# AlexandreGac/alphazero-chess

Measured on NVIDIA B200. Metric: mcts_simulations_per_sec, higher is better.
Workload: dtype bf16

## Files before the change

### alphazero-chess_b200/csrc/mcts.cu

```cuda
#include "mcts.h"
#include "nn.h"
#include "det_math.cuh"
#include <cstdio>
#include <cstring>
#include <algorithm>
#include <cmath>

namespace azb {

constexpr int WARPS = 4;

struct WarpShared {
    double gam[AZ_MAX_MOVES];
    float fval[AZ_MAX_MOVES];
    uint16_t moves[AZ_MAX_MOVES];
    uint16_t sidx[AZ_MAX_MOVES];
    DPos child;
    DPos key;
    int n_moves;
    int term;
    int has_ep;
    int pad;
};

__device__ __forceinline__ u64 rng_u64(u64 seed, u64 game, u64 ply, u64 stream, u64 counter) {
// ... 544 lines not shown
    move_step(x);
    return ColdOut{x.c, x.st_pos, x.st_games, x.st_sdepth};
}
__device__ __noinline__ ColdOut finish_game_cold(const SearchParams* prm, const SearchPtrs* ptr, WarpShared* sh, int g, GameCtl c) {
    Ctx x = cold_ctx(prm, ptr, sh, g, c);
    finish_game(x, __uint_as_float(c.park_scale));
    return ColdOut{x.c, x.st_pos, x.st_games, x.st_sdepth};
}
__device__ __noinline__ void root_noise_cold(const SearchParams* prm, const SearchPtrs* ptr, WarpShared* sh, int g, GameCtl c) {
    Ctx x = cold_ctx(prm, ptr, sh, g, c);
    apply_noise(x, 0, c.game_id, c.noise_ply);
}

#ifdef AZ_ADV_TIMING
#define ADV_T0() long long t_prev = clock64(), t_start = t_prev; unsigned long long t_acc[8] = {0, 0, 0, 0, 0, 0, 0, 0}
#define ADV_T(k) do { const long long t_now = clock64(); t_acc[k] += (unsigned long long)(t_now - t_prev); t_prev = t_now; } while (0)
#else
#define ADV_T0() do { } while (0)
#define ADV_T(k) do { } while (0)
#endif
template <int MINB>
__global__ void __launch_bounds__(WARPS * 32, MINB * 4 / WARPS) k_advance(const __grid_constant__ SearchParams prm, const __grid_constant__ SearchPtrs ptr) {
    __shared__ WarpShared shared[WARPS];
    const int g = (blockIdx.x * blockDim.x + threadIdx.x) >> 5;
    if (g >= prm.n_games) return;
    const uint2 path_spec = ptr.path[(size_t)g * prm.node_cap + min((int)(threadIdx.x & 31), prm.node_cap - 1)];
    Ctx x{prm, ptr, &shared[threadIdx.x >> 5], g, (int)(threadIdx.x & 31), (size_t)g * prm.node_cap, (size_t)g * prm.edge_cap,
          ptr.ctl[g], 0, 0, 0, 0, 0, 0, 0, 0, 0, 0, 0};
    if (g == 0 && x.lane == 0 && ptr.batch_zero) *ptr.batch_zero = 0;
    if (x.c.status != 0 && x.c.status != 4) return;
    if (!prm.consume && x.c.pending_node >= 0) return;

    ADV_T0();
    if (x.c.status == 4) {
        const ColdOut o = finish_game_cold(&prm, &ptr, x.sh, g, x.c);
        x.c = o.c; x.st_pos += o.st_pos; x.st_games += o.st_games; x.st_sdepth += o.st_sdepth;
    }
    const bool runnable = x.c.status == 0;
    if (runnable && x.c.pending_node >= 0) {
        const int node = x.c.pending_node, slot = x.c.pending_slot;
        const size_t off = x.ebase + ptr.node_edge_off[x.nbase + node];
        const int L = ptr.node_nedges[x.nbase + node];
        if (!prm.priors_scattered) {
            const float* pol = ptr.res_policy + (size_t)slot * AZ_ACTION_SPACE;
            for (int e = x.lane; e < L; e += 32) ptr.edge_P[off + e] = pol[ptr.edge_mv[off + e] >> 16];
        }
// ... 512 lines not shown
}

static void prof_mark_search(az_engine* e) {
    if (e->prof_every > 0 && e->stub_kind == 0 && e->cfg.precision != 1 && (e->prof_counter % (uint64_t)e->prof_every) == 0 &&
        !e->prof_adv_event) {
        cudaEventCreate(&e->prof_adv_event);
        cudaEventRecord(e->prof_adv_event, e->stream);
    }
}

static int run_wave(az_engine* e, SearchState* st) {
    const int blocks = (st->prm.n_games + WARPS - 1) / WARPS;
    st->prm.priors_scattered = (e->stub_kind == 0 && e->cfg.precision != 1) ? 1 : 0;
    if (st->prm.mode == 1) st->prm.cache_epoch = (uint32_t)((st->wave_counter++ / (unsigned long long)std::max(st->prm.S, 1)) & 63);
    st->batch_parity ^= 1;
    st->ptr.batch_count = st->batch_base + st->batch_parity;
    st->ptr.batch_zero = st->batch_base + (st->batch_parity ^ 1);
    prof_mark_search(e);
    const int passes = st->prm.mode == 1 && st->prm.cache_mask ? st->adv_passes : 1;
    for (int pass = 0; pass < passes; pass++) {
    st->prm.consume = pass == 0 ? 1 : 0;
    e->n_launches++;
    const int minb = e->knobs.adv_minb;
    switch (minb) {
        case 4: k_advance<4><<<blocks, WARPS * 32, 0, e->stream>>>(st->prm, st->ptr); break;
        case 5: k_advance<5><<<blocks, WARPS * 32, 0, e->stream>>>(st->prm, st->ptr); break;
        case 6: k_advance<6><<<blocks, WARPS * 32, 0, e->stream>>>(st->prm, st->ptr); break;
        case 7: k_advance<7><<<blocks, WARPS * 32, 0, e->stream>>>(st->prm, st->ptr); break;
        default: k_advance<3><<<blocks, WARPS * 32, 0, e->stream>>>(st->prm, st->ptr); break;
    }
    }
    st->prm.consume = 1;
    AZ_CUDA(e, cudaGetLastError());
    return evaluate_batch(e, st);
}

static int search_begin(az_engine* e, int n, const az_position* roots, const az_position* history, const uint32_t* hist_offsets,
                        int num_simulations, const uint64_t* noise_game_ids, const uint32_t* noise_plies, const float* visits_out,
                        SearchState& run) {
    SearchState* st = e->search;
    if (n < 0 || n > st->G) return set_err(e, AZ_ERR_CAPACITY, "more roots than az_config.max_games");
    if (n == 0) return 1;
    if (!roots || !visits_out) return set_err(e, AZ_ERR_INVALID_ARGUMENT, "null buffer");
    if (num_simulations <= 0 || num_simulations + 2 > st->prm.node_cap)
        return set_err(e, AZ_ERR_CAPACITY, "num_simulations exceeds az_config.num_simulations (pool size)");
    if (e->stub_kind == 0 && !e->net->loaded) return set_err(e, AZ_ERR_NO_WEIGHTS, "az_load_weights has not been called");
    cudaSetDevice(e->cfg.device);
    st->selfplay_active = false;
    SearchParams prm = st->prm;
    prm.n_games = n; prm.S = num_simulations; prm.mode = 0;
    run = *st;
    run.prm = prm;
    AZ_CUDA(e, cudaMemcpyAsync(e->d_wire, roots, (size_t)n * sizeof(az_position), cudaMemcpyHostToDevice, e->stream));
// ... 339 lines not shown
```

### alphazero-chess_b200/csrc/nn_heads_tc.cu

```cuda
#include "nn.h"
#include "tc_conv.cuh"
#include "device_once.h"
#include <algorithm>

namespace azb {
namespace htc {
constexpr int kStages = 3;
constexpr int kStageBytes = 32768;
constexpr int kOffA = 0;
constexpr int kW40Block = 48 * 128;
constexpr int kOffW40 = kOffA + kStages * kStageBytes;
constexpr int kOffW2 = kOffW40 + 2 * kW40Block;
constexpr int kOffP1 = kOffW2 + 64 * 64;
constexpr int kOffExp = kOffP1 + 2 * 8192;
constexpr int kV1Pitch = 520;
constexpr int kOffV1 = kOffExp + 4 * 16384;
constexpr int kOffMisc = kOffV1 + 32 * kV1Pitch * 2;
constexpr int kTotal = kOffMisc + 1024 + 1024;
constexpr int kGroupTiles = 16;
constexpr int kEpiThreads = 512;
constexpr int kThreads = 64 + kEpiThreads;
constexpr int kTmemCols = 512;
static_assert(kOffW40 % 1024 == 0 && kOffW2 % 1024 == 0 && kOffP1 % 1024 == 0 && kOffExp % 1024 == 0, "operand tiles must be 1024-byte aligned");
static_assert(kTotal <= 232448, "shared memory of one CTA");
// ... 83 lines not shown
    uint32_t* tmem_ptr_s = reinterpret_cast<uint32_t*>(wl1_full + 1);
    float* s_b40 = reinterpret_cast<float*>(misc + 160);
    float* s_b2 = reinterpret_cast<float*>(misc + 320);
    float* s_red = reinterpret_cast<float*>(misc + 576);
    float* s_vsum = reinterpret_cast<float*>(misc + 704);
    __nv_bfloat16* s_v1 = reinterpret_cast<__nv_bfloat16*>(smem + kOffV1);
    float* s_hid = reinterpret_cast<float*>(smem + kOffExp);

#ifdef AZ_HTC_TIMING
    long long tacc[20] = {}, tlast = clock64();
    const long long tbegin = tlast;
#endif
    const int t = threadIdx.x, warp = t >> 5, lane = t & 31;
    uint4 wreg[2] = {make_uint4(0, 0, 0, 0), make_uint4(0, 0, 0, 0)}, w2reg = make_uint4(0, 0, 0, 0);
#pragma unroll
    for (int u = 0; u < 2; u++) {
        const int i = t + u * kThreads;
        if (i < 40 * 16) wreg[u] = __ldg(reinterpret_cast<const uint4*>(w40) + i);
    }
    if (t < 64 * 4) w2reg = __ldg(reinterpret_cast<const uint4*>(wp2) + t);
    float breg = 0.0f;
    if (t < 40) breg = b40[t];
    else if (t >= 64 && t < 128) breg = bp2[t - 64];
    const int n = n_dev ? *n_dev : n_static;
    const int n_tiles = (n + 1) >> 1;
    const int my_tiles = (int)blockIdx.x < n_tiles ? (n_tiles - (int)blockIdx.x + (int)gridDim.x - 1) / (int)gridDim.x : 0;

    const int et = t - 64;
    const int ew = warp - 2;
    const int w = ew >> 3;
    const int q = warp & 3;
    const int cg = (ew & 7) >> 2;
    const int row = q * 32 + lane;
    const int bi = q >> 1, sq = row & 63;
    const int ti = (q & 1) + 2 * cg;
    const int tid128 = sq + 64 * cg;
    const int nw = (my_tiles - w + 1) >> 1;
    unsigned long long eo_cur = 0, eo_nxt = 0, eo_n2 = 0;
    int L_cur = 0, L_nxt = 0, L_n2 = 0;
    uint32_t mv_cur = 0, mv_nxt = 0;
    auto meta = [&](int j, unsigned long long& eo, int& L) {
        eo = 0; L = 0;
        if (sc.edge_P && j < nw) {
            const int b = ((int)blockIdx.x + (2 * j + w) * (int)gridDim.x) * 2 + bi;
            if (b < n) { eo = sc.edge_off[b]; L = sc.n_edges[b]; }
        }
    };
    if (warp >= 2) { meta(0, eo_cur, L_cur); meta(1, eo_nxt, L_nxt); }

    if (t == 0) {
        tma_prefetch_desc(&act_map);
        for (int i = 0; i < kStages; i++) { mbar_init(&a_full[i], 1); mbar_init(&a_empty[i], 1); }
        for (int i = 0; i < 2; i++) { mbar_init(&d1_full[i], 1); mbar_init(&p1_ready[i], 8); }
        for (int i = 0; i < 4; i++) { mbar_init(&d2_full[i], 1); mbar_init(&d2_free[i], 8); }
        mbar_init(wl1_full, 1);
        fence_barrier_init();
        for (int k = 0; k < kStages && k < my_tiles; k++) {
            const int tile = (int)blockIdx.x + k * (int)gridDim.x;
            mbar_arrive_expect_tx(&a_full[k], kStageBytes);
            tma1_load_2d(smem + kOffA + k * kStageBytes, &act_map, &a_full[k], 0, tile * 128);
            tma1_load_2d(smem + kOffA + k * kStageBytes + 16384, &act_map, &a_full[k], 64, tile * 128);
        }
    }
#pragma unroll
    for (int u = 0; u < 2; u++) {
        const int i = t + u * kThreads;
        if (i < 48 * 16) {
            const int r = i >> 4, ch = i & 15;
            *reinterpret_cast<uint4*>(smem + kOffW40 + (ch >> 3) * kW40Block + (r >> 3) * 1024 + (r & 7) * 128 + (((ch & 7) ^ (r & 7)) << 4)) = wreg[u];
        }
    }
    if (t < 64 * 4) {
        const int r = t >> 2, c = t & 3;
        *reinterpret_cast<uint4*>(smem + kOffW2 + (r >> 3) * 512 + (r & 7) * 64 + ((c ^ ((r >> 1) & 3)) << 4)) = w2reg;
    }
    if (t < 40) s_b40[t] = breg;
    if (t >= 64 && t < 128) s_b2[t - 64] = breg;
    fence_proxy_async_smem();
    if (warp == 1) tmem1_alloc(tmem_ptr_s, kTmemCols);
    tc_fence_before();
    __syncthreads();
    tc_fence_after();
    const uint32_t tmem_base = *tmem_ptr_s;
    HTC_T(0);

    if (warp == 0) {
        int stage = 0; uint32_t phase = 1;
        for (int k = kStages; k < my_tiles; k++) {
            const int tile = (int)blockIdx.x + k * (int)gridDim.x;
            mbar_wait(&a_empty[stage], phase ^ 1, 21);
            HTC_T(1);
            if (elect_one()) {
                mbar_arrive_expect_tx(&a_full[stage], kStageBytes);
                tma1_load_2d(smem + kOffA + stage * kStageBytes, &act_map, &a_full[stage], 0, tile * 128);
                tma1_load_2d(smem + kOffA + stage * kStageBytes + 16384, &act_map, &a_full[stage], 64, tile * 128);
            }
            __syncwarp();
            if (++stage == kStages) { stage = 0; phase ^= 1; }
        }
        if (my_tiles > 0 && my_tiles <= kGroupTiles) {
            for (int i = 0; i < kStages && i < my_tiles; i++) {
                mbar_wait(&a_empty[stage], phase ^ 1, 28);
                if (++stage == kStages) { stage = 0; phase ^= 1; }
            }
            if (elect_one()) {
                mbar_arrive_expect_tx(wl1_full, 64 * 1024);
// ... 220 lines not shown
    }
#ifdef AZ_HTC_TIMING
    if (blockIdx.x == 0 && lane == 0 && (warp <= 2 || warp == 10)) {
        const long long tot = clock64() - tbegin;
        printf("htc warp %d total %lld | setup %lld | p1 %lld p2 %lld p3 %lld p4 %lld p5 %lld p6 %lld p7 %lld p8 %lld p9 %lld p10 %lld p11 %lld p12 %lld p13 %lld p14 %lld p15 %lld | exp %lld shfl %lld\n", warp, tot,
               tacc[0], tacc[1], tacc[2], tacc[3], tacc[4], tacc[5], tacc[6], tacc[7], tacc[8], tacc[9], tacc[10], tacc[11], tacc[12], tacc[13], tacc[14], tacc[15], tacc[16], tacc[17]);
    }
#endif
    tc_fence_before();
    __syncthreads();
    if (warp == 1) { tc_fence_after(); tmem1_dealloc(tmem_base, kTmemCols); }
}

int launch_heads_tc(az_engine* e, const CUtensorMap* act_map, const int* n_dev, int n_static, float* policy_out, float* value_out,
                    const HeadScatter* scatter) {
    NetWeights* w = e->net;
    const int n_max = n_dev ? w->max_boards : n_static;
    if (n_max <= 0) return 0;
    const int grid = std::min((n_max + 1) / 2, e->sm_count);
    static PerDeviceOnce once;
    if (once.first()) cudaFuncSetAttribute(k_heads_tc, cudaFuncAttributeMaxDynamicSharedMemorySize, htc::kTotal);
    HeadScatter sc{nullptr, nullptr, nullptr, nullptr};
    if (scatter) sc = *scatter;
    k_heads_tc<<<grid, htc::kThreads, htc::kTotal, e->stream>>>(*act_map, w->h_w40, w->f_b40, w->h_wp2, w->f_bp2, w->h_wl1t, w->f_bl1, w->f_wl2,
                                                               w->f_bl2, policy_out, value_out, n_dev, n_static, sc);
    return check_cuda(e, cudaGetLastError(), "k_heads_tc");
}

}
```

### alphazero-chess_b200/csrc/nn_tc.cu

```cuda
#include "tc_conv.cuh"
#include "nn_tc.h"
#include "device_once.h"
#include <cuda_bf16.h>
#include <cstdio>
#include <cstdlib>

namespace azb {

constexpr int kWTileBytes = 64 * 128;

template <int HALVES, int KROW = 128, int WIDE = 0>
struct ConvSmem {
    static constexpr int kPitch = WIDE == 1 ? 16 : WIDE == 2 ? 10 : 8;
    static constexpr int kStages = HALVES == 1 ? 6 : WIDE == 1 ? 2 : WIDE == 2 ? 3 : 4;
    static constexpr int kWTiles = HALVES * 9;
    static constexpr int kStageB = 20 * kPitch * KROW;
    static constexpr int kWTileB = 64 * KROW;
    static constexpr int kWBytes = kWTiles * kWTileB;
    static constexpr int kABytes = kStages * kStageB;
    static constexpr int kMisc = 2048;
    static constexpr int kTotal = kWBytes + kABytes + kMisc + 1024;
};

constexpr int kTmemCols2 = 256;
// ... 11 lines not shown
__global__ void __cluster_dims__(2, 1, 1) __launch_bounds__(64 + GROUPS * kEpiThreads, 1)
conv3x3_tc2_kernel(const __grid_constant__ CUtensorMap in_map, const __grid_constant__ CUtensorMap w_map,
                   const float* __restrict__ bias, const __nv_bfloat16* __restrict__ residual,
                   __nv_bfloat16* __restrict__ out, const int* __restrict__ n_boards_ptr, int n_boards_static, int relu, int dbg) {
    using S = ConvSmem<HALVES, KROW, WIDE>;
    constexpr int kStageBytes = S::kStageB, kWTileBytes = S::kWTileB;
    constexpr int KSTEPS = KROW / 32;
    constexpr int NS = S::kStages;
    extern __shared__ uint8_t smem_raw[];
    uint8_t* smem = reinterpret_cast<uint8_t*>((reinterpret_cast<uintptr_t>(smem_raw) + 1023) & ~uintptr_t(1023));
    uint8_t* w_sm = smem;
    uint8_t* a_sm = smem + S::kWBytes;
    uint8_t* misc = a_sm + S::kABytes;
    float* bias_s = reinterpret_cast<float*>(misc);
    uint64_t* full_bar = reinterpret_cast<uint64_t*>(misc + 512);
    uint64_t* empty_bar = full_bar + NS;
    uint64_t* wfull_bar = empty_bar + NS;
    uint64_t* tfull_bar = wfull_bar + S::kWTiles;
    uint64_t* tempty_bar = tfull_bar + 2;
    uint32_t* tmem_ptr_s = reinterpret_cast<uint32_t*>(tempty_bar + 2);

    const int warp = threadIdx.x >> 5, lane = threadIdx.x & 31;
    const uint32_t rank = cluster_ctarank();
    const int n_boards = n_boards_ptr ? *n_boards_ptr : n_boards_static;
    const int n_tiles = (n_boards + 3) >> 2;
    const int first_tile = blockIdx.x >> 1, tile_step = gridDim.x >> 1;

    if (threadIdx.x == 0) {
        tma_prefetch_desc(&in_map);
        tma_prefetch_desc(&w_map);
        for (int i = 0; i < NS; i++) { mbar_init(&full_bar[i], 1); mbar_init(&empty_bar[i], 1); }
        for (int i = 0; i < S::kWTiles; i++) mbar_init(&wfull_bar[i], 1);
        for (int i = 0; i < 2; i++) { mbar_init(&tfull_bar[i], 1); mbar_init(&tempty_bar[i], 2 * kEpiWarps); }
        fence_barrier_init();
    }
    if (threadIdx.x >= 64 && threadIdx.x < 192) bias_s[threadIdx.x - 64] = bias[threadIdx.x - 64];
    if (warp == 1) tmem2_alloc(tmem_ptr_s, kTmemCols2);
    tc_fence_before();
    __syncthreads();
    cluster_sync_all();
    tc_fence_after();
    const uint32_t tmem_base = *tmem_ptr_s;

    if (warp == 0) {
        int stage = 0; uint32_t phase = 0; bool first = true;
        for (int t = first_tile; t < n_tiles; t += tile_step) {
            if constexpr (WIDE) {
                for (int half = 0; half < HALVES; half++) {
                    if (first && elect_one()) {
                        for (int dxi = 0; dxi < 3; dxi++)
                            for (int dyi = 0; dyi < 3; dyi++) {
                                const int wt = (half * 3 + dxi) * 3 + dyi, tap = dyi * 3 + dxi;
                                if (rank == 0) mbar_arrive_expect_tx(&wfull_bar[wt], 2 * kWTileBytes);
                                tma2_load_2d(w_sm + wt * kWTileBytes, &w_map, &wfull_bar[wt], half * 64, tap * 128 + (int)rank * 64);
                            }
                    }
                    mbar_wait(&empty_bar[stage], phase ^ 1, 11);
                    if (elect_one()) {
                        if (rank == 0) mbar_arrive_expect_tx(&full_bar[stage], 2 * kStageBytes);
                        tma2_load_4d(a_sm + stage * kStageBytes, &in_map, &full_bar[stage], half * 64, -1, t * 4 + (int)rank * 2, -1);
                    }
                    __syncwarp();
                    if (++stage == NS) { stage = 0; phase ^= 1; }
                }
                first = false;
            } else {
            for (int half = 0; half < HALVES; half++)
                for (int dxi = 0; dxi < 3; dxi++) {
                    if (first && elect_one()) {
                        for (int dyi = 0; dyi < 3; dyi++) {
                            const int wt = (half * 3 + dxi) * 3 + dyi, tap = dyi * 3 + dxi;
                            if (rank == 0) mbar_arrive_expect_tx(&wfull_bar[wt], 2 * kWTileBytes);
                            tma2_load_2d(w_sm + wt * kWTileBytes, &w_map, &wfull_bar[wt], half * 64, tap * 128 + (int)rank * 64);
                        }
                    }
                    mbar_wait(&empty_bar[stage], phase ^ 1, 11);
                    if (elect_one()) {
                        if (dbg & 1) { if (rank == 0) mbar_arrive(&full_bar[stage]); }
                        else {
                            if (rank == 0) mbar_arrive_expect_tx(&full_bar[stage], 2 * kStageBytes);
                            tma2_load_4d(a_sm + stage * kStageBytes, &in_map, &full_bar[stage], half * 64, dxi - 1, t * 4 + (int)rank * 2, -1);
                        }
                    }
                    __syncwarp();
                    if (++stage == NS) { stage = 0; phase ^= 1; }
                }
            first = false;
            }
        }
    } else if (warp == 1) {
        if (rank == 0) {
            constexpr uint32_t idesc = umma_idesc_bf16(256, 128);
            const uint64_t dbase = KROW == 128 ? umma_desc_base_sw128() : umma_desc_base_sw64();
            const uint32_t w_lo = (smem_u32(w_sm) & 0x3FFFF) >> 4;
            int stage = 0; uint32_t phase = 0; int lt = 0;
            for (int t = first_tile; t < n_tiles; t += tile_step, lt++) {
                const int acc = lt & 1; const uint32_t accphase = (lt >> 1) & 1;
                mbar_wait(&tempty_bar[acc], accphase ^ 1, 12);
                tc_fence_after();
                const uint32_t d_tmem = tmem_base + acc * 128;
                if constexpr (WIDE) {
                    for (int half = 0; half < HALVES; half++) {
                        mbar_wait(&full_bar[stage], phase, 13);
                        if (lt == 0)
                            for (int wt = 0; wt < 9; wt++) mbar_wait(&wfull_bar[half * 9 + wt], 0, 14);
                        tc_fence_after();
                        if (elect_one()) {
                            const uint32_t a_lo = (smem_u32(a_sm + stage * kStageBytes) & 0x3FFFF) >> 4;
                            const uint64_t abase = ((uint64_t)1 << 16) | ((uint64_t)((S::kPitch * KROW) >> 4) << 32) | ((uint64_t)1 << 46) | ((uint64_t)(KROW == 128 ? 2 : 4) << 61);
#pragma unroll
                            for (int dxi = 0; dxi < 3; dxi++) {
                                const uint32_t b_lo = w_lo + (uint32_t)((half * 3 + dxi) * 3) * (kWTileBytes >> 4);
// ... 132 lines not shown
template <int WIDE>
__global__ void __cluster_dims__(2, 1, 1) __launch_bounds__(kThreads2, 1)
conv_tower_kernel(const TowerParams prm) {
    using S = ConvSmem<2, 128, WIDE>;
    constexpr int kStageBytes = S::kStageB;
    constexpr int NS = S::kStages;
    constexpr int kGroupBytes = 3 * kWTileBytes;
    extern __shared__ uint8_t smem_raw[];
    uint8_t* smem = reinterpret_cast<uint8_t*>((reinterpret_cast<uintptr_t>(smem_raw) + 1023) & ~uintptr_t(1023));
    uint8_t* w_sm = smem;
    uint8_t* a_sm = smem + S::kWBytes;
    uint8_t* misc = a_sm + S::kABytes;
    uint64_t* full_bar = reinterpret_cast<uint64_t*>(misc);
    uint64_t* empty_bar = full_bar + NS;
    uint64_t* wfull_bar = empty_bar + NS;
    uint64_t* wempty_bar = wfull_bar + 6;
    uint64_t* tfull_bar = wempty_bar + 6;
    uint64_t* tempty_bar = tfull_bar + 2;
    uint32_t* tmem_ptr_s = reinterpret_cast<uint32_t*>(tempty_bar + 2);
    volatile uint32_t* epi_done = reinterpret_cast<volatile uint32_t*>(tmem_ptr_s + 4);

    const int warp = threadIdx.x >> 5, lane = threadIdx.x & 31;
    const uint32_t rank = cluster_ctarank();
    const int n_boards = prm.n_boards_ptr ? *prm.n_boards_ptr : prm.n_boards_static;
    const int n_tiles = min((n_boards + 3) >> 2, prm.tile_hi);
    const int tile_step = gridDim.x >> 1;
    const int n_ranges = n_tiles > prm.tile_lo ? (n_tiles - prm.tile_lo + prm.range_tiles - 1) / prm.range_tiles : 0;
#define TOWER_RANGE_BEGIN()                                                                                      \
    const int range_lo = prm.tile_lo + rg * prm.range_tiles;                                                      \
    const int range_hi = min(n_tiles, range_lo + prm.range_tiles);                                               \
    const int first_tile = range_lo + (blockIdx.x >> 1);                                                         \
    const int T = first_tile < range_hi ? (range_hi - first_tile + tile_step - 1) / tile_step : 0;               \
    if (T == 0) continue;
    const int stem = prm.stem;
    const int NL = prm.n_layers + stem;

    if (threadIdx.x == 0) {
        for (int i = 0; i < NS; i++) { mbar_init(&full_bar[i], 1); mbar_init(&empty_bar[i], 1); }
        for (int i = 0; i < 6; i++) { mbar_init(&wfull_bar[i], 1); mbar_init(&wempty_bar[i], 1); }
        for (int i = 0; i < 2; i++) { mbar_init(&tfull_bar[i], 1); mbar_init(&tempty_bar[i], 2 * kEpiWarps); }
        fence_barrier_init();
    }
    if (threadIdx.x < kEpiWarps) epi_done[threadIdx.x] = 0;
    float* bias_s = reinterpret_cast<float*>(misc + 512);
    if (warp == 1) tmem2_alloc(tmem_ptr_s, kTmemCols2);
    tc_fence_before();
    __syncthreads();
    cluster_sync_all();
    tc_fence_after();
    const uint32_t tmem_base = *tmem_ptr_s;

    if (warp == 0) {
        int stage = 0; uint32_t phase = 0;
        int u0 = 0, u1 = 0;
        uint32_t cum = 0;
        for (int rg = 0; rg < n_ranges; rg++) {
        TOWER_RANGE_BEGIN();
        for (int L = 0; L < NL; L++) {
            const int layer = L - stem;
            const int blk_second = layer >= 0 ? (layer & 1) : 0;
            const int in_buf = blk_second ? 1 : 0;
            const CUtensorMap* in_map = layer >= 0 ? &prm.maps[(WIDE == 2 ? 28 : WIDE ? 25 : 0) + in_buf] : &prm.maps[23];
            const CUtensorMap* w_map = layer >= 0 ? &prm.maps[3 + layer] : &prm.maps[24];
            const int halves = layer >= 0 ? 2 : 1;
            for (int i = 0; i < T; i++) {
                const int t = first_tile + i * tile_step;
                if (L > 0) {
                    const uint32_t need = cum + (uint32_t)((L - 1) * T + i + 1);
                    long long t0 = clock64();
                    for (;;) {
                        bool ok = lane >= kEpiWarps || epi_done[lane & (kEpiWarps - 1)] >= need;
                        if (__all_sync(0xffffffffu, ok)) break;
                        if (clock64() - t0 > 4000000000LL) { if (lane == 0) printf("azb: tower epilogue wait timeout\n"); __trap(); }
                    }
                    fence_proxy_async();
                }
                for (int half = 0; half < halves; half++)
                    for (int dxi = 0; dxi < 3; dxi++) {
                        const int grp = half * 3 + dxi;
                        if (i == 0) {
                            const int used = half == 0 ? u0 : u1;
                            if (used > 0) mbar_wait(&wempty_bar[grp], (uint32_t)((used - 1) & 1), 21);
                            if (elect_one()) {
                                if (rank == 0) mbar_arrive_expect_tx(&wfull_bar[grp], 2 * kGroupBytes);
                                for (int dyi = 0; dyi < 3; dyi++)
                                    tma2_load_2d(w_sm + (grp * 3 + dyi) * kWTileBytes, w_map, &wfull_bar[grp], half * 64,
                                                 (dyi * 3 + dxi) * 128 + (int)rank * 64);
                            }
                            __syncwarp();
                        }
                        if (WIDE && dxi != 2) continue;
                        mbar_wait(&empty_bar[stage], phase ^ 1, 22);
                        if (elect_one()) {
                            if (rank == 0) mbar_arrive_expect_tx(&full_bar[stage], 2 * kStageBytes);
                            if (prm.l2_hint & 4) tma2_load_4d_hint(a_sm + stage * kStageBytes, in_map, &full_bar[stage], half * 64, WIDE ? -1 : dxi - 1, t * 4 + (int)rank * 2, -1, l2_policy_evict_last());
                            else tma2_load_4d(a_sm + stage * kStageBytes, in_map, &full_bar[stage], half * 64, WIDE ? -1 : dxi - 1, t * 4 + (int)rank * 2, -1);
                        }
                        __syncwarp();
                        if (++stage == NS) { stage = 0; phase ^= 1; }
                    }
            }
            u0++;
            if (halves == 2) u1++;
        }
        cum += (uint32_t)(NL * T);
        }
    } else if (warp == 1) {
        if (rank == 0) {
            constexpr uint32_t idesc = umma_idesc_bf16(256, 128);
            const uint64_t dbase = umma_desc_base_sw128();
            const uint32_t w_lo = (smem_u32(w_sm) & 0x3FFFF) >> 4;
            int stage = 0; uint32_t phase = 0; int lt = 0;
            int u0 = 0, u1 = 0;
            for (int rg = 0; rg < n_ranges; rg++) {
            TOWER_RANGE_BEGIN();
            for (int L = 0; L < NL; L++) {
                const int layer = L - stem;
                const int halves = layer >= 0 ? 2 : 1;
                for (int i = 0; i < T; i++, lt++) {
                    const int acc = lt & 1; const uint32_t accphase = (lt >> 1) & 1;
                    mbar_wait(&tempty_bar[acc], accphase ^ 1, 23);
                    tc_fence_after();
                    const uint32_t d_tmem = tmem_base + acc * 128;
                    for (int half = 0; half < halves; half++)
                        for (int dxi = 0; dxi < 3; dxi++) {
                            const int grp = half * 3 + dxi;
                            if (!WIDE || dxi == 0) mbar_wait(&full_bar[stage], phase, 24);
                            if (i == 0) mbar_wait(&wfull_bar[grp], (uint32_t)((half == 0 ? u0 : u1) & 1), 25);
                            tc_fence_after();
// ... 119 lines not shown
    cluster_sync_all();
    if (warp == 1) { tc_fence_after(); tmem2_dealloc(tmem_base, kTmemCols2); }
}

int tc_tower_launch(cudaStream_t stream, const CUtensorMap* maps_dev, const float* bias, void* const* act, const int* n_boards_dev,
                    int n_boards_static, int n_layers, int stem, int grid, int tile_lo, int tile_hi, int range_tiles, int release_arrive,
                    int wide, int l2_hint) {
    static PerDeviceOnce once;
    if (once.first() &&
        (cudaFuncSetAttribute(conv_tower_kernel<0>, cudaFuncAttributeMaxDynamicSharedMemorySize, ConvSmem<2>::kTotal) != cudaSuccess ||
         cudaFuncSetAttribute(conv_tower_kernel<1>, cudaFuncAttributeMaxDynamicSharedMemorySize, ConvSmem<2, 128, 1>::kTotal) != cudaSuccess ||
         cudaFuncSetAttribute(conv_tower_kernel<2>, cudaFuncAttributeMaxDynamicSharedMemorySize, ConvSmem<2, 128, 2>::kTotal) != cudaSuccess))
        return -2;
    if (wide && stem) return -5;
    if (grid <= 0) grid = 148;
    grid &= ~1;
    TowerParams p;
    p.maps = maps_dev; p.bias = bias;
    for (int i = 0; i < 3; i++) p.act[i] = (__nv_bfloat16*)act[i];
    p.n_boards_ptr = n_boards_dev; p.n_boards_static = n_boards_static; p.n_layers = n_layers; p.stem = stem ? 1 : 0;
    p.tile_lo = tile_lo; p.tile_hi = tile_hi; p.range_tiles = range_tiles > 0 ? range_tiles : (1 << 30);
    p.release_arrive = release_arrive;
    p.l2_hint = l2_hint;
    if (wide == 2) conv_tower_kernel<2><<<grid, kThreads2, ConvSmem<2, 128, 2>::kTotal, stream>>>(p);
    else if (wide) conv_tower_kernel<1><<<grid, kThreads2, ConvSmem<2, 128, 1>::kTotal, stream>>>(p);
    else conv_tower_kernel<0><<<grid, kThreads2, ConvSmem<2>::kTotal, stream>>>(p);
    return cudaGetLastError() == cudaSuccess ? 0 : -4;
}

typedef CUresult (*PFN_encodeTiled)(CUtensorMap*, CUtensorMapDataType, cuuint32_t, void*, const cuuint64_t*, const cuuint64_t*,
                                    const cuuint32_t*, const cuuint32_t*, CUtensorMapInterleave, CUtensorMapSwizzle,
                                    CUtensorMapL2promotion, CUtensorMapFloatOOBfill);

static PFN_encodeTiled get_encode() {
    static PFN_encodeTiled fn = nullptr;
    if (!fn) {
        void* p = nullptr;
        cudaDriverEntryPointQueryResult qres;
        if (cudaGetDriverEntryPoint("cuTensorMapEncodeTiled", &p, cudaEnableDefault, &qres) != cudaSuccess || !p) return nullptr;
        fn = reinterpret_cast<PFN_encodeTiled>(p);
    }
    return fn;
}

int tc_make_act_map(CUtensorMap* map, const void* base, int channels, int max_boards, int wide) {
    PFN_encodeTiled enc = get_encode();
    if (!enc) return -1;
    cuuint64_t dims[4] = {(cuuint64_t)channels, 8, (cuuint64_t)max_boards, 8};
    cuuint64_t strides[3] = {(cuuint64_t)channels * 2, (cuuint64_t)channels * 2 * 64, (cuuint64_t)channels * 2 * 8};
    cuuint32_t box[4] = {(cuuint32_t)(channels == 32 ? 32 : 64), (cuuint32_t)(wide == 1 ? 16 : wide == 2 ? 10 : 8), 2, 10};
// ... 25 lines not shown
    cuuint32_t box[2] = {(cuuint32_t)(cin == 32 ? 32 : 64), 64};
    cuuint32_t estr[2] = {1, 1};
    CUresult r = enc(map, CU_TENSOR_MAP_DATA_TYPE_BFLOAT16, 2, const_cast<void*>(base), dims, strides, box, estr,
                     CU_TENSOR_MAP_INTERLEAVE_NONE, cin == 32 ? CU_TENSOR_MAP_SWIZZLE_64B : CU_TENSOR_MAP_SWIZZLE_128B, CU_TENSOR_MAP_L2_PROMOTION_L2_256B,
                     CU_TENSOR_MAP_FLOAT_OOB_FILL_NONE);
    return r == CUDA_SUCCESS ? 0 : -(int)r - 1000;
}

int tc_conv3x3_launch(cudaStream_t stream, const CUtensorMap* in_map, const CUtensorMap* w_map, int cin, const float* bias,
                      const void* residual, void* out, const int* n_boards_dev, int n_boards_static, int relu, int grid, int dbg) {
    static PerDeviceOnce once;
    if (once.first()) {
        cudaError_t e1 = cudaFuncSetAttribute(conv3x3_tc2_kernel<1, 128>, cudaFuncAttributeMaxDynamicSharedMemorySize, ConvSmem<1>::kTotal);
        cudaError_t e2 = cudaFuncSetAttribute(conv3x3_tc2_kernel<2, 128>, cudaFuncAttributeMaxDynamicSharedMemorySize, ConvSmem<2>::kTotal);
        cudaError_t e3 = cudaFuncSetAttribute(conv3x3_tc2_kernel<1, 64>, cudaFuncAttributeMaxDynamicSharedMemorySize, ConvSmem<1, 64>::kTotal);
        cudaError_t e4 = cudaFuncSetAttribute(conv3x3_tc2_kernel<2, 128, 1>, cudaFuncAttributeMaxDynamicSharedMemorySize, ConvSmem<2, 128, 1>::kTotal);
        cudaError_t e5 = cudaFuncSetAttribute(conv3x3_tc2_kernel<2, 128, 2>, cudaFuncAttributeMaxDynamicSharedMemorySize, ConvSmem<2, 128, 2>::kTotal);
        cudaError_t e6 = cudaFuncSetAttribute(conv3x3_tc2_kernel<1, 64, 2>, cudaFuncAttributeMaxDynamicSharedMemorySize, ConvSmem<1, 64, 2>::kTotal);
        cudaError_t e7 = cudaFuncSetAttribute(conv3x3_tc2_kernel<1, 64, 0, 2>, cudaFuncAttributeMaxDynamicSharedMemorySize, ConvSmem<1, 64>::kTotal);
        if (e1 != cudaSuccess || e2 != cudaSuccess || e3 != cudaSuccess || e4 != cudaSuccess || e5 != cudaSuccess || e6 != cudaSuccess || e7 != cudaSuccess) return -2;
    }
    if (grid <= 0) grid = 148;
    grid &= ~1;
    if (cin == 32 && (dbg & 256))
        conv3x3_tc2_kernel<1, 64, 2><<<grid, kThreads2, ConvSmem<1, 64, 2>::kTotal, stream>>>(*in_map, *w_map, bias, (const __nv_bfloat16*)residual,
                                                                                            (__nv_bfloat16*)out, n_boards_dev, n_boards_static, relu, dbg);
    else if (cin == 32 && (dbg & 1024))
        conv3x3_tc2_kernel<1, 64, 0, 2><<<grid, 64 + 2 * kEpiThreads, ConvSmem<1, 64>::kTotal, stream>>>(*in_map, *w_map, bias, (const __nv_bfloat16*)residual,
                                                                                                  (__nv_bfloat16*)out, n_boards_dev, n_boards_static, relu, dbg);
    else if (cin == 32)
        conv3x3_tc2_kernel<1, 64><<<grid, kThreads2, ConvSmem<1, 64>::kTotal, stream>>>(*in_map, *w_map, bias, (const __nv_bfloat16*)residual,
                                                                                       (__nv_bfloat16*)out, n_boards_dev, n_boards_static, relu, dbg);
    else if (cin == 64)
        conv3x3_tc2_kernel<1, 128><<<grid, kThreads2, ConvSmem<1>::kTotal, stream>>>(*in_map, *w_map, bias, (const __nv_bfloat16*)residual,
                                                                                    (__nv_bfloat16*)out, n_boards_dev, n_boards_static, relu, dbg);
    else if (cin == 128 && (dbg & 256))
        conv3x3_tc2_kernel<2, 128, 2><<<grid, kThreads2, ConvSmem<2, 128, 2>::kTotal, stream>>>(*in_map, *w_map, bias, (const __nv_bfloat16*)residual,
                                                                                              (__nv_bfloat16*)out, n_boards_dev, n_boards_static, relu, dbg);
    else if (cin == 128 && (dbg & 64))
        conv3x3_tc2_kernel<2, 128, 1><<<grid, kThreads2, ConvSmem<2, 128, 1>::kTotal, stream>>>(*in_map, *w_map, bias, (const __nv_bfloat16*)residual,
                                                                                              (__nv_bfloat16*)out, n_boards_dev, n_boards_static, relu, dbg);
    else if (cin == 128)
        conv3x3_tc2_kernel<2, 128><<<grid, kThreads2, ConvSmem<2>::kTotal, stream>>>(*in_map, *w_map, bias, (const __nv_bfloat16*)residual,
                                                                                    (__nv_bfloat16*)out, n_boards_dev, n_boards_static, relu, dbg);
    else
        return -3;
    return cudaGetLastError() == cudaSuccess ? 0 : -4;
}

}
```

Baseline: 3.725 million.

## Enable programmatic dependent launch across advance, conv and head kernels

New measurement: 3.725 million (median of 6 runs). About the same (+0.0%).

```diff
diff --git a/alphazero-chess_b200/csrc/mcts.cu b/alphazero-chess_b200/csrc/mcts.cu
--- a/alphazero-chess_b200/csrc/mcts.cu
+++ b/alphazero-chess_b200/csrc/mcts.cu
@@ -1,6 +1,7 @@
 #include "mcts.h"
 #include "nn.h"
 #include "det_math.cuh"
+#include "pdl.cuh"
 #include <cstdio>
 #include <cstring>
 #include <algorithm>
@@ -591,6 +592,8 @@
 template <int MINB>
 __global__ void __launch_bounds__(WARPS * 32, MINB * 4 / WARPS) k_advance(const __grid_constant__ SearchParams prm, const __grid_constant__ SearchPtrs ptr) {
     __shared__ WarpShared shared[WARPS];
+    pdl_wait();
+    pdl_launch_dependents();
     const int g = (blockIdx.x * blockDim.x + threadIdx.x) >> 5;
     if (g >= prm.n_games) return;
     const uint2 path_spec = ptr.path[(size_t)g * prm.node_cap + min((int)(threadIdx.x & 31), prm.node_cap - 1)];
@@ -1149,13 +1152,8 @@
     st->prm.consume = pass == 0 ? 1 : 0;
     e->n_launches++;
     const int minb = e->knobs.adv_minb;
-    switch (minb) {
-        case 4: k_advance<4><<<blocks, WARPS * 32, 0, e->stream>>>(st->prm, st->ptr); break;
-        case 5: k_advance<5><<<blocks, WARPS * 32, 0, e->stream>>>(st->prm, st->ptr); break;
-        case 6: k_advance<6><<<blocks, WARPS * 32, 0, e->stream>>>(st->prm, st->ptr); break;
-        case 7: k_advance<7><<<blocks, WARPS * 32, 0, e->stream>>>(st->prm, st->ptr); break;
-        default: k_advance<3><<<blocks, WARPS * 32, 0, e->stream>>>(st->prm, st->ptr); break;
-    }
+    auto* kernel = minb == 4 ? k_advance<4> : minb == 5 ? k_advance<5> : minb == 6 ? k_advance<6> : minb == 7 ? k_advance<7> : k_advance<3>;
+    AZ_CUDA(e, launch_pdl(kernel, blocks, WARPS * 32, 0, e->stream, st->prm, st->ptr));
     }
     st->prm.consume = 1;
     AZ_CUDA(e, cudaGetLastError());
diff --git a/alphazero-chess_b200/csrc/nn_heads_tc.cu b/alphazero-chess_b200/csrc/nn_heads_tc.cu
--- a/alphazero-chess_b200/csrc/nn_heads_tc.cu
+++ b/alphazero-chess_b200/csrc/nn_heads_tc.cu
@@ -1,5 +1,6 @@
 #include "nn.h"
 #include "tc_conv.cuh"
+#include "pdl.cuh"
 #include "device_once.h"
 #include <algorithm>
 
@@ -129,9 +130,48 @@
     float breg = 0.0f;
     if (t < 40) breg = b40[t];
     else if (t >= 64 && t < 128) breg = bp2[t - 64];
+    if (t == 0) {
+        tma_prefetch_desc(&act_map);
+        for (int i = 0; i < kStages; i++) { mbar_init(&a_full[i], 1); mbar_init(&a_empty[i], 1); }
+        for (int i = 0; i < 2; i++) { mbar_init(&d1_full[i], 1); mbar_init(&p1_ready[i], 8); }
+        for (int i = 0; i < 4; i++) { mbar_init(&d2_full[i], 1); mbar_init(&d2_free[i], 8); }
+        mbar_init(wl1_full, 1);
+        fence_barrier_init();
+    }
+#pragma unroll
+    for (int u = 0; u < 2; u++) {
+        const int i = t + u * kThreads;
+        if (i < 48 * 16) {
+            const int r = i >> 4, ch = i & 15;
+            *reinterpret_cast<uint4*>(smem + kOffW40 + (ch >> 3) * kW40Block + (r >> 3) * 1024 + (r & 7) * 128 + (((ch & 7) ^ (r & 7)) << 4)) = wreg[u];
+        }
+    }
+    if (t < 64 * 4) {
+        const int r = t >> 2, c = t & 3;
+        *reinterpret_cast<uint4*>(smem + kOffW2 + (r >> 3) * 512 + (r & 7) * 64 + ((c ^ ((r >> 1) & 3)) << 4)) = w2reg;
+    }
+    if (t < 40) s_b40[t] = breg;
+    if (t >= 64 && t < 128) s_b2[t - 64] = breg;
+    fence_proxy_async_smem();
+    if (warp == 1) tmem1_alloc(tmem_ptr_s, kTmemCols);
+    tc_fence_before();
+    __syncthreads();
+    tc_fence_after();
+    const uint32_t tmem_base = *tmem_ptr_s;
+    pdl_launch_dependents();
+    pdl_wait();
+
     const int n = n_dev ? *n_dev : n_static;
     const int n_tiles = (n + 1) >> 1;
     const int my_tiles = (int)blockIdx.x < n_tiles ? (n_tiles - (int)blockIdx.x + (int)gridDim.x - 1) / (int)gridDim.x : 0;
+    if (t == 0) {
+        for (int k = 0; k < kStages && k < my_tiles; k++) {
+            const int tile = (int)blockIdx.x + k * (int)gridDim.x;
+            mbar_arrive_expect_tx(&a_full[k], kStageBytes);
+            tma1_load_2d(smem + kOffA + k * kStageBytes, &act_map, &a_full[k], 0, tile * 128);
+            tma1_load_2d(smem + kOffA + k * kStageBytes + 16384, &act_map, &a_full[k], 64, tile * 128);
+        }
+    }
 
     const int et = t - 64;
     const int ew = warp - 2;
@@ -154,41 +194,6 @@
         }
     };
     if (warp >= 2) { meta(0, eo_cur, L_cur); meta(1, eo_nxt, L_nxt); }
-
-    if (t == 0) {
-        tma_prefetch_desc(&act_map);
-        for (int i = 0; i < kStages; i++) { mbar_init(&a_full[i], 1); mbar_init(&a_empty[i], 1); }
-        for (int i = 0; i < 2; i++) { mbar_init(&d1_full[i], 1); mbar_init(&p1_ready[i], 8); }
-        for (int i = 0; i < 4; i++) { mbar_init(&d2_full[i], 1); mbar_init(&d2_free[i], 8); }
-        mbar_init(wl1_full, 1);
-        fence_barrier_init();
-        for (int k = 0; k < kStages && k < my_tiles; k++) {
-            const int tile = (int)blockIdx.x + k * (int)gridDim.x;
-            mbar_arrive_expect_tx(&a_full[k], kStageBytes);
-            tma1_load_2d(smem + kOffA + k * kStageBytes, &act_map, &a_full[k], 0, tile * 128);
-            tma1_load_2d(smem + kOffA + k * kStageBytes + 16384, &act_map, &a_full[k], 64, tile * 128);
-        }
-    }
-#pragma unroll
-    for (int u = 0; u < 2; u++) {
-        const int i = t + u * kThreads;
-        if (i < 48 * 16) {
-            const int r = i >> 4, ch = i & 15;
-            *reinterpret_cast<uint4*>(smem + kOffW40 + (ch >> 3) * kW40Block + (r >> 3) * 1024 + (r & 7) * 128 + (((ch & 7) ^ (r & 7)) << 4)) = wreg[u];
-        }
-    }
-    if (t < 64 * 4) {
-        const int r = t >> 2, c = t & 3;
-        *reinterpret_cast<uint4*>(smem + kOffW2 + (r >> 3) * 512 + (r & 7) * 64 + ((c ^ ((r >> 1) & 3)) << 4)) = w2reg;
-    }
-    if (t < 40) s_b40[t] = breg;
-    if (t >= 64 && t < 128) s_b2[t - 64] = breg;
-    fence_proxy_async_smem();
-    if (warp == 1) tmem1_alloc(tmem_ptr_s, kTmemCols);
-    tc_fence_before();
-    __syncthreads();
-    tc_fence_after();
-    const uint32_t tmem_base = *tmem_ptr_s;
     HTC_T(0);
 
     if (warp == 0) {
@@ -455,9 +460,9 @@
     if (once.first()) cudaFuncSetAttribute(k_heads_tc, cudaFuncAttributeMaxDynamicSharedMemorySize, htc::kTotal);
     HeadScatter sc{nullptr, nullptr, nullptr, nullptr};
     if (scatter) sc = *scatter;
-    k_heads_tc<<<grid, htc::kThreads, htc::kTotal, e->stream>>>(*act_map, w->h_w40, w->f_b40, w->h_wp2, w->f_bp2, w->h_wl1t, w->f_bl1, w->f_wl2,
-                                                               w->f_bl2, policy_out, value_out, n_dev, n_static, sc);
-    return check_cuda(e, cudaGetLastError(), "k_heads_tc");
-}
-
-}
+    return check_cuda(e, launch_pdl(k_heads_tc, grid, htc::kThreads, htc::kTotal, e->stream, *act_map, w->h_w40, w->f_b40, w->h_wp2, w->f_bp2,
+                                    w->h_wl1t, w->f_bl1, w->f_wl2, w->f_bl2, policy_out, value_out, n_dev, n_static, sc),
+                      "k_heads_tc");
+}
+
+}
diff --git a/alphazero-chess_b200/csrc/nn_tc.cu b/alphazero-chess_b200/csrc/nn_tc.cu
--- a/alphazero-chess_b200/csrc/nn_tc.cu
+++ b/alphazero-chess_b200/csrc/nn_tc.cu
@@ -1,4 +1,5 @@
 #include "tc_conv.cuh"
+#include "pdl.cuh"
 #include "nn_tc.h"
 #include "device_once.h"
 #include <cuda_bf16.h>
@@ -57,8 +58,6 @@
 
     const int warp = threadIdx.x >> 5, lane = threadIdx.x & 31;
     const uint32_t rank = cluster_ctarank();
-    const int n_boards = n_boards_ptr ? *n_boards_ptr : n_boards_static;
-    const int n_tiles = (n_boards + 3) >> 2;
     const int first_tile = blockIdx.x >> 1, tile_step = gridDim.x >> 1;
 
     if (threadIdx.x == 0) {
@@ -76,20 +75,23 @@
     cluster_sync_all();
     tc_fence_after();
     const uint32_t tmem_base = *tmem_ptr_s;
+    if (warp == 0 && elect_one()) {
+        for (int wt = 0; wt < S::kWTiles; wt++) {
+            const int half = wt / 9, dxi = (wt / 3) % 3, dyi = wt % 3, tap = dyi * 3 + dxi;
+            if (rank == 0) mbar_arrive_expect_tx(&wfull_bar[wt], 2 * kWTileBytes);
+            tma2_load_2d(w_sm + wt * kWTileBytes, &w_map, &wfull_bar[wt], half * 64, tap * 128 + (int)rank * 64);
+        }
+    }
+    pdl_launch_dependents();
+    pdl_wait();
+    const int n_boards = n_boards_ptr ? *n_boards_ptr : n_boards_static;
+    const int n_tiles = (n_boards + 3) >> 2;
 
     if (warp == 0) {
-        int stage = 0; uint32_t phase = 0; bool first = true;
+        int stage = 0; uint32_t phase = 0;
         for (int t = first_tile; t < n_tiles; t += tile_step) {
             if constexpr (WIDE) {
                 for (int half = 0; half < HALVES; half++) {
-                    if (first && elect_one()) {
-                        for (int dxi = 0; dxi < 3; dxi++)
-                            for (int dyi = 0; dyi < 3; dyi++) {
-                                const int wt = (half * 3 + dxi) * 3 + dyi, tap = dyi * 3 + dxi;
-                                if (rank == 0) mbar_arrive_expect_tx(&wfull_bar[wt], 2 * kWTileBytes);
-                                tma2_load_2d(w_sm + wt * kWTileBytes, &w_map, &wfull_bar[wt], half * 64, tap * 128 + (int)rank * 64);
-                            }
-                    }
                     mbar_wait(&empty_bar[stage], phase ^ 1, 11);
                     if (elect_one()) {
                         if (rank == 0) mbar_arrive_expect_tx(&full_bar[stage], 2 * kStageBytes);
@@ -98,17 +100,9 @@
                     __syncwarp();
                     if (++stage == NS) { stage = 0; phase ^= 1; }
                 }
-                first = false;
             } else {
             for (int half = 0; half < HALVES; half++)
                 for (int dxi = 0; dxi < 3; dxi++) {
-                    if (first && elect_one()) {
-                        for (int dyi = 0; dyi < 3; dyi++) {
-                            const int wt = (half * 3 + dxi) * 3 + dyi, tap = dyi * 3 + dxi;
-                            if (rank == 0) mbar_arrive_expect_tx(&wfull_bar[wt], 2 * kWTileBytes);
-                            tma2_load_2d(w_sm + wt * kWTileBytes, &w_map, &wfull_bar[wt], half * 64, tap * 128 + (int)rank * 64);
-                        }
-                    }
                     mbar_wait(&empty_bar[stage], phase ^ 1, 11);
                     if (elect_one()) {
                         if (dbg & 1) { if (rank == 0) mbar_arrive(&full_bar[stage]); }
@@ -120,9 +114,10 @@
                     __syncwarp();
                     if (++stage == NS) { stage = 0; phase ^= 1; }
                 }
-            first = false;
-            }
-        }
+            }
+        }
+        if (first_tile >= n_tiles && rank == 0)
+            for (int wt = 0; wt < S::kWTiles; wt++) mbar_wait(&wfull_bar[wt], 0, 14);
     } else if (warp == 1) {
         if (rank == 0) {
             constexpr uint32_t idesc = umma_idesc_bf16(256, 128);
@@ -301,10 +296,7 @@
 
     const int warp = threadIdx.x >> 5, lane = threadIdx.x & 31;
     const uint32_t rank = cluster_ctarank();
-    const int n_boards = prm.n_boards_ptr ? *prm.n_boards_ptr : prm.n_boards_static;
-    const int n_tiles = min((n_boards + 3) >> 2, prm.tile_hi);
     const int tile_step = gridDim.x >> 1;
-    const int n_ranges = n_tiles > prm.tile_lo ? (n_tiles - prm.tile_lo + prm.range_tiles - 1) / prm.range_tiles : 0;
 #define TOWER_RANGE_BEGIN()                                                                                      \
     const int range_lo = prm.tile_lo + rg * prm.range_tiles;                                                      \
     const int range_hi = min(n_tiles, range_lo + prm.range_tiles);                                               \
@@ -328,6 +320,21 @@
     cluster_sync_all();
     tc_fence_after();
     const uint32_t tmem_base = *tmem_ptr_s;
+    const int first_groups = stem ? 3 : 6;
+    if (warp == 0 && elect_one()) {
+        const CUtensorMap* w_map0 = stem ? &prm.maps[24] : &prm.maps[3];
+        for (int grp = 0; grp < first_groups; grp++) {
+            const int half = grp / 3, dxi = grp % 3;
+            if (rank == 0) mbar_arrive_expect_tx(&wfull_bar[grp], 2 * kGroupBytes);
+            for (int dyi = 0; dyi < 3; dyi++)
+                tma2_load_2d(w_sm + (grp * 3 + dyi) * kWTileBytes, w_map0, &wfull_bar[grp], half * 64, (dyi * 3 + dxi) * 128 + (int)rank * 64);
+        }
+    }
+    pdl_launch_dependents();
+    pdl_wait();
+    const int n_boards = prm.n_boards_ptr ? *prm.n_boards_ptr : prm.n_boards_static;
+    const int n_tiles = min((n_boards + 3) >> 2, prm.tile_hi);
+    const int n_ranges = n_tiles > prm.tile_lo ? (n_tiles - prm.tile_lo + prm.range_tiles - 1) / prm.range_tiles : 0;
 
     if (warp == 0) {
         int stage = 0; uint32_t phase = 0;
@@ -357,7 +364,7 @@
                 for (int half = 0; half < halves; half++)
                     for (int dxi = 0; dxi < 3; dxi++) {
                         const int grp = half * 3 + dxi;
-                        if (i == 0) {
+                        if (i == 0 && u0 > 0) {
                             const int used = half == 0 ? u0 : u1;
                             if (used > 0) mbar_wait(&wempty_bar[grp], (uint32_t)((used - 1) & 1), 21);
                             if (elect_one()) {
@@ -384,6 +391,8 @@
         }
         cum += (uint32_t)(NL * T);
         }
+        if (u0 == 0 && rank == 0)
+            for (int grp = 0; grp < first_groups; grp++) mbar_wait(&wfull_bar[grp], 0, 21);
     } else if (warp == 1) {
         if (rank == 0) {
             constexpr uint32_t idesc = umma_idesc_bf16(256, 128);
@@ -549,10 +558,11 @@
     p.tile_lo = tile_lo; p.tile_hi = tile_hi; p.range_tiles = range_tiles > 0 ? range_tiles : (1 << 30);
     p.release_arrive = release_arrive;
     p.l2_hint = l2_hint;
-    if (wide == 2) conv_tower_kernel<2><<<grid, kThreads2, ConvSmem<2, 128, 2>::kTotal, stream>>>(p);
-    else if (wide) conv_tower_kernel<1><<<grid, kThreads2, ConvSmem<2, 128, 1>::kTotal, stream>>>(p);
-    else conv_tower_kernel<0><<<grid, kThreads2, ConvSmem<2>::kTotal, stream>>>(p);
-    return cudaGetLastError() == cudaSuccess ? 0 : -4;
+    cudaError_t r;
+    if (wide == 2) r = launch_pdl(conv_tower_kernel<2>, grid, kThreads2, ConvSmem<2, 128, 2>::kTotal, stream, p);
+    else if (wide) r = launch_pdl(conv_tower_kernel<1>, grid, kThreads2, ConvSmem<2, 128, 1>::kTotal, stream, p);
+    else r = launch_pdl(conv_tower_kernel<0>, grid, kThreads2, ConvSmem<2>::kTotal, stream, p);
+    return r == cudaSuccess ? 0 : -4;
 }
 
 typedef CUresult (*PFN_encodeTiled)(CUtensorMap*, CUtensorMapDataType, cuuint32_t, void*, const cuuint64_t*, const cuuint64_t*,
@@ -624,30 +634,31 @@
     }
     if (grid <= 0) grid = 148;
     grid &= ~1;
+    cudaError_t r;
     if (cin == 32 && (dbg & 256))
-        conv3x3_tc2_kernel<1, 64, 2><<<grid, kThreads2, ConvSmem<1, 64, 2>::kTotal, stream>>>(*in_map, *w_map, bias, (const __nv_bfloat16*)residual,
-                                                                                            (__nv_bfloat16*)out, n_boards_dev, n_boards_static, relu, dbg);
+        r = launch_pdl(conv3x3_tc2_kernel<1, 64, 2>, grid, kThreads2, ConvSmem<1, 64, 2>::kTotal, stream, *in_map, *w_map, bias, (const __nv_bfloat16*)residual,
+                       (__nv_bfloat16*)out, n_boards_dev, n_boards_static, relu, dbg);
     else if (cin == 32 && (dbg & 1024))
-        conv3x3_tc2_kernel<1, 64, 0, 2><<<grid, 64 + 2 * kEpiThreads, ConvSmem<1, 64>::kTotal, stream>>>(*in_map, *w_map, bias, (const __nv_bfloat16*)residual,
-                                                                                                  (__nv_bfloat16*)out, n_boards_dev, n_boards_static, relu, dbg);
+        r = launch_pdl(conv3x3_tc2_kernel<1, 64, 0, 2>, grid, 64 + 2 * kEpiThreads, ConvSmem<1, 64>::kTotal, stream, *in_map, *w_map, bias, (const __nv_bfloat16*)residual,
+                       (__nv_bfloat16*)out, n_boards_dev, n_boards_static, relu, dbg);
     else if (cin == 32)
-        conv3x3_tc2_kernel<1, 64><<<grid, kThreads2, ConvSmem<1, 64>::kTotal, stream>>>(*in_map, *w_map, bias, (const __nv_bfloat16*)residual,
-                                                                                       (__nv_bfloat16*)out, n_boards_dev, n_boards_static, relu, dbg);
+        r = launch_pdl(conv3x3_tc2_kernel<1, 64>, grid, kThreads2, ConvSmem<1, 64>::kTotal, stream, *in_map, *w_map, bias, (const __nv_bfloat16*)residual,
+                       (__nv_bfloat16*)out, n_boards_dev, n_boards_static, relu, dbg);
     else if (cin == 64)
-        conv3x3_tc2_kernel<1, 128><<<grid, kThreads2, ConvSmem<1>::kTotal, stream>>>(*in_map, *w_map, bias, (const __nv_bfloat16*)residual,
-                                                                                    (__nv_bfloat16*)out, n_boards_dev, n_boards_static, relu, dbg);
+        r = launch_pdl(conv3x3_tc2_kernel<1, 128>, grid, kThreads2, ConvSmem<1>::kTotal, stream, *in_map, *w_map, bias, (const __nv_bfloat16*)residual,
+                       (__nv_bfloat16*)out, n_boards_dev, n_boards_static, relu, dbg);
     else if (cin == 128 && (dbg & 256))
-        conv3x3_tc2_kernel<2, 128, 2><<<grid, kThreads2, ConvSmem<2, 128, 2>::kTotal, stream>>>(*in_map, *w_map, bias, (const __nv_bfloat16*)residual,
-                                                                                              (__nv_bfloat16*)out, n_boards_dev, n_boards_static, relu, dbg);
+        r = launch_pdl(conv3x3_tc2_kernel<2, 128, 2>, grid, kThreads2, ConvSmem<2, 128, 2>::kTotal, stream, *in_map, *w_map, bias, (const __nv_bfloat16*)residual,
+                       (__nv_bfloat16*)out, n_boards_dev, n_boards_static, relu, dbg);
     else if (cin == 128 && (dbg & 64))
-        conv3x3_tc2_kernel<2, 128, 1><<<grid, kThreads2, ConvSmem<2, 128, 1>::kTotal, stream>>>(*in_map, *w_map, bias, (const __nv_bfloat16*)residual,
-                                                                                              (__nv_bfloat16*)out, n_boards_dev, n_boards_static, relu, dbg);
+        r = launch_pdl(conv3x3_tc2_kernel<2, 128, 1>, grid, kThreads2, ConvSmem<2, 128, 1>::kTotal, stream, *in_map, *w_map, bias, (const __nv_bfloat16*)residual,
+                       (__nv_bfloat16*)out, n_boards_dev, n_boards_static, relu, dbg);
     else if (cin == 128)
-        conv3x3_tc2_kernel<2, 128><<<grid, kThreads2, ConvSmem<2>::kTotal, stream>>>(*in_map, *w_map, bias, (const __nv_bfloat16*)residual,
-                                                                                    (__nv_bfloat16*)out, n_boards_dev, n_boards_static, relu, dbg);
+        r = launch_pdl(conv3x3_tc2_kernel<2, 128>, grid, kThreads2, ConvSmem<2>::kTotal, stream, *in_map, *w_map, bias, (const __nv_bfloat16*)residual,
+                       (__nv_bfloat16*)out, n_boards_dev, n_boards_static, relu, dbg);
     else
         return -3;
-    return cudaGetLastError() == cudaSuccess ? 0 : -4;
-}
-
-}
+    return r == cudaSuccess ? 0 : -4;
+}
+
+}
diff --git a/alphazero-chess_b200/csrc/pdl.cuh b/alphazero-chess_b200/csrc/pdl.cuh
--- /dev/null
+++ b/alphazero-chess_b200/csrc/pdl.cuh
@@ -0,0 +1,25 @@
+#pragma once
+#include <cuda_runtime.h>
+#include <utility>
+
+namespace azb {
+
+__device__ __forceinline__ void pdl_wait() { asm volatile("griddepcontrol.wait;" ::: "memory"); }
+__device__ __forceinline__ void pdl_launch_dependents() { asm volatile("griddepcontrol.launch_dependents;" ::: "memory"); }
+
+template <typename... KArgs, typename... Args>
+cudaError_t launch_pdl(void (*kernel)(KArgs...), dim3 grid, dim3 block, size_t smem, cudaStream_t stream, Args&&... args) {
+    cudaLaunchAttribute attr[1];
+    attr[0].id = cudaLaunchAttributeProgrammaticStreamSerialization;
+    attr[0].val.programmaticStreamSerializationAllowed = 1;
+    cudaLaunchConfig_t cfg = {};
+    cfg.gridDim = grid;
+    cfg.blockDim = block;
+    cfg.dynamicSmemBytes = smem;
+    cfg.stream = stream;
+    cfg.attrs = attr;
+    cfg.numAttrs = 1;
+    return cudaLaunchKernelEx(&cfg, kernel, std::forward<Args>(args)...);
+}
+
+}
```
